# teoremma/pgen-rs

Hardware: AMD Instinct MI355X
Metric: genotypes decoded/sec (variants x samples / s) (higher is better)
Workload: dtype u8

## Files before the change

include/pgen_hip.h:

```cpp
#ifndef PGEN_HIP_H
#define PGEN_HIP_H

#include <stddef.h>
#include <stdint.h>

#ifdef __cplusplus
extern "C" {
#endif

#define PGENHIP_ABI_VERSION 2u
#define PGENHIP_LAUNCHES_IN_FLIGHT 16u

typedef enum pgenhip_status {
    PGENHIP_OK = 0,
    PGENHIP_ERR_BAD_ARG = -1,
    PGENHIP_ERR_HIP = -2,
    PGENHIP_ERR_OOM = -3,
    PGENHIP_ERR_INDEX_RANGE = -4,
    PGENHIP_ERR_BAD_MAGIC = -5,
    PGENHIP_ERR_BAD_MODE = -6,
    PGENHIP_ERR_BAD_FLAGS = -7,
    PGENHIP_ERR_NO_DEVICE = -8,
    PGENHIP_ERR_TOO_LARGE = -9,
    PGENHIP_ERR_IO = -10,
// ... 59 lines not shown

int pgenhip_decode_emit_at(pgenhip_ctx *ctx, const void *d_base, const uint64_t *d_record_off, uint32_t n_variants,
                           void *d_out, uint64_t out_stride, uint32_t flags);

int pgenhip_emit_lines(pgenhip_ctx *ctx, const void *d_records, uint64_t record_stride,
                       const uint32_t *d_variant_idx, uint32_t n_variants,
                       const void *d_prefix_blob, const uint64_t *d_prefix_off,
                       const uint64_t *d_line_off, uint64_t max_prefix_bytes,
                       void *d_out, uint32_t flags);

#define PGENHIP_COUNT_AUTO 0u
#define PGENHIP_COUNT_WAVE_PER_ROW 1u
#define PGENHIP_COUNT_ROWS_PER_WAVE 2u
int pgenhip_genotype_counts(pgenhip_ctx *ctx, const void *d_records, uint64_t record_stride, const uint32_t *d_variant_idx,
                            uint32_t n_variants, uint32_t *d_counts, uint32_t flags);
int pgenhip_genotype_counts_at(pgenhip_ctx *ctx, const void *d_base, const uint64_t *d_record_off, uint32_t n_variants,
                               uint32_t *d_counts, uint32_t flags);

#define PGENHIP_SCOUNT_AUTO 0u
#define PGENHIP_SCOUNT_ROWS 2u
#define PGENHIP_SCOUNT_SHAPE_MASK 0xFu
#define PGENHIP_SCOUNT_ACCUMULATE 0x10u
int pgenhip_sample_counts(pgenhip_ctx *ctx, const void *d_records, uint64_t record_stride, const uint32_t *d_variant_idx,
                          uint32_t n_variants, uint32_t *d_counts, uint32_t flags);
int pgenhip_sample_counts_at(pgenhip_ctx *ctx, const void *d_base, const uint64_t *d_record_off, uint32_t n_variants,
                             uint32_t *d_counts, uint32_t flags);

#define PGENHIP_MATRIX_AUTO 0u
#define PGENHIP_MATRIX_GENERAL 1u
#define PGENHIP_MATRIX_STREAM 2u
#define PGENHIP_MATRIX_TILE 3u
#define PGENHIP_MATRIX_SHAPE_MASK 0xFu
#define PGENHIP_MATRIX_SAMPLE_MAJOR 0x10u
int pgenhip_decode_matrix(pgenhip_ctx *ctx, const void *d_records, uint64_t record_stride, const uint32_t *d_variant_idx,
                          uint32_t n_variants, void *d_out, uint64_t out_stride, uint32_t elem_bytes,
                          const void *code_values, uint32_t flags);
int pgenhip_decode_matrix_at(pgenhip_ctx *ctx, const void *d_base, const uint64_t *d_record_off, uint32_t n_variants,
                             void *d_out, uint64_t out_stride, uint32_t elem_bytes, const void *code_values, uint32_t flags);

typedef enum pgenhip_knob {
    PGENHIP_KNOB_WIDE_BLOCKS_PER_CU = 1,
    PGENHIP_KNOB_WIDE_RANGES = 2,
    PGENHIP_KNOB_FLAT_BLOCKS_PER_CU = 3,
    PGENHIP_KNOB_SCAN_BLOCKS_PER_CU = 4,
    PGENHIP_KNOB_PICK_BATCH_BYTES = 6,
    PGENHIP_KNOB_SCAN_XCD_MAP = 8,
    PGENHIP_KNOB_SCAN_TWO_PASS = 9,
    PGENHIP_KNOB_SCAN_CHUNK_ROWS = 10,
    PGENHIP_KNOB_ROWPICK_BLOCKS_PER_CU = 11,
    PGENHIP_KNOB_SCAN_ROWPICK = 12,
    PGENHIP_KNOB_ALIGN_STORES = 16,
    PGENHIP_KNOB_SCOUNT_SLICES = 17,
    PGENHIP_KNOB_MATRIX_BLOCKS = 18,
    PGENHIP_KNOB_RUNS_ROWS = 7
} pgenhip_knob;
int pgenhip_tune(pgenhip_ctx *ctx, uint32_t knob, int32_t value);

int pgenhip_wait(pgenhip_ctx *ctx);

int pgenhip_timer_start(pgenhip_ctx *ctx);
int pgenhip_timer_stop(pgenhip_ctx *ctx, float *elapsed_ms);
int pgenhip_timer_mark(pgenhip_ctx *ctx);
int pgenhip_timer_read(pgenhip_ctx *ctx, float *elapsed_ms);

int pgenhip_device_malloc(pgenhip_ctx *ctx, void **d_ptr, size_t bytes);
int pgenhip_device_free(pgenhip_ctx *ctx, void *d_ptr);
int pgenhip_host_malloc_pinned(pgenhip_ctx *ctx, void **h_ptr, size_t bytes);
int pgenhip_host_free_pinned(pgenhip_ctx *ctx, void *h_ptr);
int pgenhip_memcpy_h2d(pgenhip_ctx *ctx, void *d_dst, const void *h_src, size_t bytes);
int pgenhip_memcpy_d2h(pgenhip_ctx *ctx, void *h_dst, const void *d_src, size_t bytes);

#define PGENHIP_SYNTH_DIRTY_PAD 1u
#define PGENHIP_SYNTH_HWE 2u
int pgenhip_synth_records(pgenhip_ctx *ctx, void *d_dst, uint64_t record_stride,
                          uint64_t first_variant, uint32_t n_variants,
                          uint64_t seed, uint32_t flags);

#ifdef __cplusplus
}
#endif
#endif
```

pgen_rs_amd/_capi.py:

```python
from __future__ import annotations

import ctypes as C
from pathlib import Path

import torch

PKG_DIR = Path(__file__).resolve().parent
LIB_PATH = PKG_DIR / "libpgen_hip.so"

OK = 0
ERR_BAD_ARG = -1
ERR_HIP = -2
ERR_OOM = -3
ERR_INDEX_RANGE = -4
ERR_BAD_MAGIC = -5
ERR_BAD_MODE = -6
ERR_BAD_FLAGS = -7
ERR_NO_DEVICE = -8
ERR_TOO_LARGE = -9
ERR_IO = -10
ERR_BAD_INDEX = -11
ERR_COMPRESSED_RECORD = -12

KERNEL_AUTO = 0
KERNEL_ROWS = 1
KERNEL_FLAT = 2
KERNEL_SCAN = 3
KERNEL_WIDE = 4
KERNEL_PICK = 6
KERNEL_RUNS = 7
KERNEL_ROWPICK = 8
COUNT_AUTO = 0
COUNT_WAVE_PER_ROW = 1
COUNT_ROWS_PER_WAVE = 2

SCOUNT_AUTO = 0
SCOUNT_ROWS = 2
SCOUNT_SHAPE_MASK = 0xF
SCOUNT_ACCUMULATE = 0x10
MATRIX_AUTO = 0
MATRIX_GENERAL = 1
MATRIX_STREAM = 2
MATRIX_TILE = 3
MATRIX_SHAPE_MASK = 0xF
MATRIX_SAMPLE_MAJOR = 0x10
SYNTH_DIRTY_PAD = 1
SYNTH_HWE = 2
CREATE_KEEP_LIST = 1
LAUNCHES_IN_FLIGHT = 16

KNOB_WIDE_BLOCKS_PER_CU = 1
KNOB_WIDE_RANGES = 2
KNOB_FLAT_BLOCKS_PER_CU = 3
KNOB_SCAN_BLOCKS_PER_CU = 4
KNOB_PICK_BATCH_BYTES = 6
KNOB_RUNS_ROWS = 7
KNOB_SCAN_XCD_MAP = 8
KNOB_SCAN_TWO_PASS = 9
KNOB_SCAN_CHUNK_ROWS = 10
KNOB_ROWPICK_BLOCKS_PER_CU = 11
KNOB_SCAN_ROWPICK = 12
KNOB_ALIGN_STORES = 16
KNOB_SCOUNT_SLICES = 17
KNOB_MATRIX_BLOCKS = 18



class VwHeader(C.Structure):
    _fields_ = [("variant_count", C.c_uint32), ("sample_count", C.c_uint32), ("storage_mode", C.c_uint8),
                ("record_type_bits", C.c_uint8), ("record_length_bytes", C.c_uint8), ("allele_count_bytes", C.c_uint8),
                ("provisional_ref_storage", C.c_uint8), ("reserved", C.c_uint8 * 3), ("block_count", C.c_uint64),
                ("main_header_body_offset", C.c_uint64), ("variant_records_offset", C.c_uint64)]


u8p = C.POINTER(C.c_uint8)
u32p = C.POINTER(C.c_uint32)
u64p = C.POINTER(C.c_uint64)
ctx_p = C.c_void_p

PROTOTYPES = {
    "pgenhip_abi_version": (C.c_uint32, []),
    "pgenhip_strerror": (C.c_char_p, [C.c_int]),
    "pgenhip_last_error_detail": (C.c_char_p, []),
    "pgenhip_device_count": (C.c_int, [C.POINTER(C.c_int)]),
    "pgenhip_variant_record_size": (C.c_uint32, [C.c_uint32]),
    "pgenhip_parse_header": (C.c_int, [C.c_char_p, u32p, u32p]),
    "pgenhip_record_offset": (C.c_uint64, [C.c_uint64, C.c_uint32]),
    "pgenhip_shard_range": (C.c_int, [C.c_uint64, C.c_uint32, C.c_uint32, u64p, u64p]),
    "pgenhip_vw_parse_header": (C.c_int, [C.c_char_p, C.POINTER(VwHeader)]),
    "pgenhip_vw_walk_index": (C.c_int, [C.POINTER(VwHeader), C.c_void_p, C.c_uint64, C.c_void_p, C.c_void_p, C.c_void_p]),
    "pgenhip_vw_select_uncompressed": (C.c_int, [C.c_void_p, C.c_void_p, C.c_void_p, C.c_uint32, C.c_void_p, C.c_uint32, C.c_uint32, C.c_void_p]),
    "pgenhip_create": (C.c_int, [C.POINTER(ctx_p), C.c_int, C.c_uint32, C.c_void_p, C.c_uint32, C.c_uint32]),
    "pgenhip_destroy": (C.c_int, [ctx_p]),
    "pgenhip_set_stream": (C.c_int, [ctx_p, C.c_void_p]),
    "pgenhip_reset_stream": (C.c_int, [ctx_p]),
    "pgenhip_sample_count": (C.c_uint32, [ctx_p]),
    "pgenhip_kept_count": (C.c_uint32, [ctx_p]),
    "pgenhip_gt_row_bytes": (C.c_uint64, [ctx_p]),
    "pgenhip_decode_emit": (C.c_int, [ctx_p, C.c_void_p, C.c_uint64, C.c_void_p, C.c_uint32, C.c_void_p, C.c_uint64, C.c_uint32]),
    "pgenhip_decode_emit_at": (C.c_int, [ctx_p, C.c_void_p, C.c_void_p, C.c_uint32, C.c_void_p, C.c_uint64, C.c_uint32]),
    "pgenhip_emit_lines": (C.c_int, [ctx_p, C.c_void_p, C.c_uint64, C.c_void_p, C.c_uint32, C.c_void_p, C.c_void_p, C.c_void_p, C.c_uint64, C.c_void_p, C.c_uint32]),
    "pgenhip_genotype_counts": (C.c_int, [ctx_p, C.c_void_p, C.c_uint64, C.c_void_p, C.c_uint32, C.c_void_p, C.c_uint32]),
    "pgenhip_genotype_counts_at": (C.c_int, [ctx_p, C.c_void_p, C.c_void_p, C.c_uint32, C.c_void_p, C.c_uint32]),
    "pgenhip_sample_counts": (C.c_int, [ctx_p, C.c_void_p, C.c_uint64, C.c_void_p, C.c_uint32, C.c_void_p, C.c_uint32]),
    "pgenhip_sample_counts_at": (C.c_int, [ctx_p, C.c_void_p, C.c_void_p, C.c_uint32, C.c_void_p, C.c_uint32]),
    "pgenhip_decode_matrix": (C.c_int, [ctx_p, C.c_void_p, C.c_uint64, C.c_void_p, C.c_uint32, C.c_void_p, C.c_uint64, C.c_uint32, C.c_void_p, C.c_uint32]),
    "pgenhip_decode_matrix_at": (C.c_int, [ctx_p, C.c_void_p, C.c_void_p, C.c_uint32, C.c_void_p, C.c_uint64, C.c_uint32, C.c_void_p, C.c_uint32]),
    "pgenhip_tune": (C.c_int, [ctx_p, C.c_uint32, C.c_int32]),
    "pgenhip_wait": (C.c_int, [ctx_p]),
    "pgenhip_timer_start": (C.c_int, [ctx_p]),
    "pgenhip_timer_stop": (C.c_int, [ctx_p, C.POINTER(C.c_float)]),
    "pgenhip_timer_mark": (C.c_int, [ctx_p]),
    "pgenhip_timer_read": (C.c_int, [ctx_p, C.POINTER(C.c_float)]),
    "pgenhip_device_malloc": (C.c_int, [ctx_p, C.POINTER(C.c_void_p), C.c_size_t]),
    "pgenhip_device_free": (C.c_int, [ctx_p, C.c_void_p]),
    "pgenhip_host_malloc_pinned": (C.c_int, [ctx_p, C.POINTER(C.c_void_p), C.c_size_t]),
    "pgenhip_host_free_pinned": (C.c_int, [ctx_p, C.c_void_p]),
# ... 35 lines not shown
```

pgen_rs_amd/csrc/capi.hip:

```cpp
#include "../../include/pgen_hip.h"

#include <algorithm>
#include <hip/hip_runtime.h>

#include <new>
#include <string>
#include <vector>

#include "host_pure.h"
#include "kernels.h"

using namespace pgenhip;

struct pgenhip_ctx {
    int device = 0;
    int num_cus = 256;
    uint32_t sample_count = 0;
    uint32_t record_size = 0;
    uint32_t kept_count = 0;
    bool subset = false;
    bool identity = false;
    uint32_t *d_kept = nullptr;
    uint8_t *d_count_mask = nullptr;
    uint32_t *d_scount_rank = nullptr;
// ... 616 lines not shown
        if (code_values) {
            const uint8_t *p = static_cast<const uint8_t *>(code_values) + (size_t)c * elem_bytes;
            v = 0u;
            for (uint32_t b = 0; b < elem_bytes; b++) v |= (uint32_t)p[b] << (8u * b);
        }
        a.tab[c] = v;
    }
    if (shape == PGENHIP_MATRIX_TILE && !gt_matrix_tile_applicable(a))
        return fail(PGENHIP_ERR_BAD_ARG, "PGENHIP_MATRIX_TILE needs d_out and out_stride to be multiples of 16 bytes");
    const int blocks = ctx->tune.matrix_blocks;
    if (shape == PGENHIP_MATRIX_STREAM || (shape == PGENHIP_MATRIX_AUTO && gt_matrix_stream_applicable(a)))
        HIP_TRY(launch_gt_matrix_stream(a, blocks, ctx->num_cus, ctx->stream));
    else if (shape == PGENHIP_MATRIX_TILE || (shape == PGENHIP_MATRIX_AUTO && gt_matrix_tile_applicable(a)))
        HIP_TRY(launch_gt_matrix_tile(a, blocks, ctx->num_cus, ctx->stream));
    else
        HIP_TRY(launch_gt_matrix_general(a, blocks, ctx->num_cus, ctx->stream));
    return PGENHIP_OK;
}

int pgenhip_decode_matrix(pgenhip_ctx *ctx, const void *d_records, uint64_t record_stride, const uint32_t *d_variant_idx,
                          uint32_t n_variants, void *d_out, uint64_t out_stride, uint32_t elem_bytes,
                          const void *code_values, uint32_t flags)
{
    return decode_matrix_core(ctx, d_records, record_stride, d_variant_idx, nullptr, n_variants, d_out, out_stride, elem_bytes, code_values, flags);
}

int pgenhip_decode_matrix_at(pgenhip_ctx *ctx, const void *d_base, const uint64_t *d_record_off, uint32_t n_variants,
                             void *d_out, uint64_t out_stride, uint32_t elem_bytes, const void *code_values, uint32_t flags)
{
    if (const int rc = check_record_off(ctx, d_record_off, n_variants)) return rc;
    return decode_matrix_core(ctx, d_base, 0, nullptr, d_record_off, n_variants, d_out, out_stride, elem_bytes, code_values, flags);
}

int pgenhip_tune(pgenhip_ctx *ctx, uint32_t knob, int32_t value)
{
    if (!ctx) return fail(PGENHIP_ERR_BAD_ARG, "ctx is NULL");
    const Tuning d;
    Tuning &t = ctx->tune;
    switch (knob) {
        case PGENHIP_KNOB_WIDE_BLOCKS_PER_CU: t.wide_blocks_per_cu = value > 0 ? value : d.wide_blocks_per_cu; break;
        case PGENHIP_KNOB_WIDE_RANGES:
            if (value < 0 || value > (int32_t)kMaxQueueRanges || (value & (value - 1)) != 0) return fail(PGENHIP_ERR_BAD_ARG, "ranges must be a power of two up to 64");
            t.wide_ranges = value ? value : d.wide_ranges;
            break;
        case PGENHIP_KNOB_FLAT_BLOCKS_PER_CU: t.flat_blocks_per_cu = value > 0 ? value : d.flat_blocks_per_cu; break;
        case PGENHIP_KNOB_SCAN_BLOCKS_PER_CU: t.scan_blocks_per_cu = value > 0 ? value : d.scan_blocks_per_cu; break;
        case PGENHIP_KNOB_PICK_BATCH_BYTES: t.pick_batch_bytes = value > 0 ? value : d.pick_batch_bytes; break;
        case PGENHIP_KNOB_SCAN_XCD_MAP: t.scan_xcd_map = value < 0 ? 0 : 1; break;
        case PGENHIP_KNOB_SCAN_CHUNK_ROWS: t.scan_chunk_rows = value > 0 ? value : d.scan_chunk_rows; break;
        case PGENHIP_KNOB_SCAN_TWO_PASS: t.scan_two_pass = value < 0 ? 0 : 1; break;
        case PGENHIP_KNOB_ROWPICK_BLOCKS_PER_CU: t.rowpick_blocks_per_cu = value > 0 ? value : d.rowpick_blocks_per_cu; break;
        case PGENHIP_KNOB_SCAN_ROWPICK: t.scan_rowpick = value < 0 ? 0 : 1; break;
        case PGENHIP_KNOB_ALIGN_STORES: t.align_stores = value < 0 ? 0 : 1; break;
        case PGENHIP_KNOB_RUNS_ROWS: t.runs_rows = value > 0 ? value : d.runs_rows; break;
        case PGENHIP_KNOB_SCOUNT_SLICES: t.scount_slices = value > 0 ? value : d.scount_slices; break;
        case PGENHIP_KNOB_MATRIX_BLOCKS: t.matrix_blocks = value > 0 ? value : d.matrix_blocks; break;
        default: return fail(PGENHIP_ERR_BAD_ARG, "unknown knob");
    }
    return PGENHIP_OK;
}

int pgenhip_wait(pgenhip_ctx *ctx)
{
    int rc = bind(ctx);
    if (rc) return rc;
    HIP_TRY(hipStreamSynchronize(ctx->stream));
    return PGENHIP_OK;
}

int pgenhip_timer_start(pgenhip_ctx *ctx)
{
    int rc = bind(ctx);
    if (rc) return rc;
    HIP_TRY(hipEventRecord(ctx->ev_start, ctx->stream));
    return PGENHIP_OK;
}

int pgenhip_timer_stop(pgenhip_ctx *ctx, float *elapsed_ms)
{
    int rc = bind(ctx);
    if (rc) return rc;
    if (!elapsed_ms) return fail(PGENHIP_ERR_BAD_ARG, "elapsed_ms is NULL");
    HIP_TRY(hipEventRecord(ctx->ev_stop, ctx->stream));
    HIP_TRY(hipEventSynchronize(ctx->ev_stop));
    HIP_TRY(hipEventElapsedTime(elapsed_ms, ctx->ev_start, ctx->ev_stop));
    return PGENHIP_OK;
}

int pgenhip_timer_mark(pgenhip_ctx *ctx)
{
    int rc = bind(ctx);
    if (rc) return rc;
    HIP_TRY(hipEventRecord(ctx->ev_stop, ctx->stream));
    return PGENHIP_OK;
}

int pgenhip_timer_read(pgenhip_ctx *ctx, float *elapsed_ms)
{
    int rc = bind(ctx);
    if (rc) return rc;
    if (!elapsed_ms) return fail(PGENHIP_ERR_BAD_ARG, "elapsed_ms is NULL");
    HIP_TRY(hipEventElapsedTime(elapsed_ms, ctx->ev_start, ctx->ev_stop));
    return PGENHIP_OK;
}

int pgenhip_device_malloc(pgenhip_ctx *ctx, void **d_ptr, size_t bytes)
// ... 73 lines not shown
```

pgen_rs_amd/csrc/gt_wide.hip:

```cpp
#include <algorithm>

#include "gt_common.hip.h"
#include "kernels.h"

namespace pgenhip {

namespace {

constexpr uint32_t kSpanChunks = 1024;
constexpr uint32_t kSlabBytes = 1088;
constexpr uint32_t kSlabExtra = 16;
constexpr uint32_t kDescBytes = 64;

struct WideParams {
    uint64_t row_bytes;
    uint64_t total_bytes;
    uint64_t n_items;
    uint32_t spans_per_row;
    uint32_t head;
    uint32_t n_ranges;
    uint32_t run_rows;
    uint32_t run_rec;
    uint32_t magic;
    uint32_t pfx_shift;
};

typedef uint32_t v4u __attribute__((ext_vector_type(4)));

template <bool HAS_VIDX>
__device__ __forceinline__ const uint8_t *row_record(const EmitArgs &a, uint64_t r)
{
    return HAS_VIDX ? gathered_record(a, r) : a.records + r * a.record_stride;
}

template <bool NT>
__device__ __forceinline__ void store_chunk(uint8_t *dst, const u32x4 &v)
{
    v4u t = {v.x, v.y, v.z, v.w};
    if (NT)
        __builtin_nontemporal_store(t, reinterpret_cast<v4u *>(dst));
    else
        *reinterpret_cast<v4u *>(dst) = t;
}

struct Item {
    uint64_t g0;
    uint32_t cnt;
    uint32_t lead;
    int64_t c_first;
    const uint8_t *rec;
    const uint8_t *base;
    uint32_t n_load;
    int32_t delta;
    uint64_t row;
    bool row_tail;
};

template <bool HAS_VIDX, bool LINES = false>
__device__ __forceinline__ Item make_item_at(const EmitArgs &a, const WideParams &p, uint64_t j, uint32_t k, uint64_t lines_row_start = 0ull,
                                             const uint8_t *rec_known = nullptr)
{
    Item it;
    const uint64_t S = p.row_bytes;
    const uint64_t row_start = LINES ? lines_row_start : j * S;
    const uint64_t g_first = (LINES || j == 0) ? (row_start + p.head) >> 4 : (row_start + p.head + 15ull) >> 4;
    const uint64_t g_end = (row_start + S + p.head + 15ull) >> 4;
    const int32_t row_chunks = (int32_t)(uint32_t)(g_end - g_first);
    const int32_t base_rel = (int32_t)(k * kSpanChunks) - (int32_t)((uint32_t)g_first & 63u);
    const int32_t end_rel = min(row_chunks, base_rel + (int32_t)kSpanChunks);
    const int32_t g0_rel = max(base_rel, 0);
    const int32_t row_c_first = (int32_t)((uint32_t)g_first * 16u - p.head - (uint32_t)row_start);
    it.row = j;
    it.g0 = g_first + (uint64_t)(uint32_t)g0_rel;
    it.cnt = end_rel > g0_rel ? (uint32_t)(end_rel - g0_rel) : 0u;
    it.lead = (uint32_t)(g0_rel - base_rel);
    it.row_tail = it.cnt != 0u && end_rel == row_chunks;
    it.c_first = (int64_t)row_c_first + ((int64_t)g0_rel << 4);
// ... 280 lines not shown
        for (uint32_t rr = rr_lo + lane; rr < rr_hi; rr += 64u) {
            const uint32_t e = rr * S + S - 1u;
            const uint32_t i = (uint32_t)((int32_t)e - c_first) >> 4;
            const uint32_t nl = (uint32_t)((int32_t)e - c_first) & 15u;
            const uint32_t slot = i + it.lead - g * 256u;
            const v4u x = st[slot];
            const bool has_next = rr + 1u < nrows || has_next_run;
            u32x4 y = {0u, 0u, 0u, 0u};
            if (nl < 15u && has_next) y = gt_text16_from_window((uint32_t)slab[delta + (rr + 1u) * R] << 8, -(int64_t)nl - 1);
            const uint32_t xs[4] = {x.x, x.y, x.z, x.w};
            const uint32_t ys[4] = {y.x, y.y, y.z, y.w};
            uint32_t os[4];
#pragma unroll
            for (int m = 0; m < 4; m++) {
                const int32_t nb = (int32_t)nl - 4 * m;
                const uint32_t mask = nb >= 4 ? 0xFFFFFFFFu : (nb <= 0 ? 0u : ((1u << (8 * nb)) - 1u));
                uint32_t d = (xs[m] & mask) | (ys[m] & ~mask);
                if (nb >= 0 && nb < 4) d = (d & ~(0xFFu << (8 * nb))) | (0x0Au << (8 * nb));
                os[m] = d;
            }
            if (has_next || nl == 15u) {
                st[slot] = v4u{os[0], os[1], os[2], os[3]};
            } else {
                uint8_t *const dst = chunk0 + (it.g0 + i) * 16ull;
#pragma unroll
                for (int b = 0; b < 16; b++)
                    if ((uint32_t)b <= nl) dst[b] = (uint8_t)(os[b >> 2] >> (8 * (b & 3)));
            }
        }
        __builtin_amdgcn_fence(__ATOMIC_RELEASE, "wavefront");
        __builtin_amdgcn_wave_barrier();
        __builtin_amdgcn_fence(__ATOMIC_ACQUIRE, "wavefront");
#pragma unroll
        for (uint32_t s4 = 0; s4 < 4u; s4++) {
            const uint32_t u = g * 4u + s4;
            if (u * 64u >= end) break;
            const uint32_t i = u * 64u + lane - it.lead;
            const v4u v = st[s4 * 64u + lane];
            if (i < cnt_whole && !(c_first < 0 && i == 0u)) store_chunk<NT>(span_ptr + u * 1024u, u32x4{v.x, v.y, v.z, v.w});
        }
        __builtin_amdgcn_fence(__ATOMIC_RELEASE, "wavefront");
        __builtin_amdgcn_wave_barrier();
    }
    if (c_first < 0 && it.cnt != 0u && lane < 16u && (int32_t)lane + c_first >= 0) {
        const uint32_t ob = (uint32_t)((int32_t)lane + c_first);
        const uint32_t code = ((uint32_t)slab[delta + (ob >> 4)] >> (((ob >> 2) & 3u) * 2u)) & 3u;
        chunk0[it.g0 * 16ull + lane] = (uint8_t)gt_text_byte(code, ob & 3u);
    }
}

constexpr int kRingSlots = 3;

template <int NS, bool HAS_VIDX, bool NT, bool LINES = false, int BURST = 2, bool RUNS = false>
__global__ __launch_bounds__(64 * (NS + 1)) void gt_stream_dyn_kernel(EmitArgs a, WideParams p)
{
    constexpr int RS = RUNS ? 2 : kRingSlots;
    constexpr int DS = RS + 1;
    __shared__ __attribute__((aligned(16))) uint8_t slabs[NS][RS][kSlabBytes + kSlabExtra];
    __shared__ __attribute__((aligned(16))) uint8_t s_desc[NS][DS][kDescBytes];
    __shared__ __attribute__((aligned(16))) uint8_t s_stage[RUNS ? NS : 1][RUNS ? kStageBytes : 16u];
    __shared__ uint32_t s_full[NS][RS];
    __shared__ uint32_t s_done[NS][RS];
    const uint32_t lane = threadIdx.x & 63u;
    const uint32_t wave = __builtin_amdgcn_readfirstlane(threadIdx.x >> 6);
    if (threadIdx.x < NS * RS) {
        (&s_full[0][0])[threadIdx.x] = 0u;
        (&s_done[0][0])[threadIdx.x] = 0u;
    }
    __syncthreads();
    constexpr uint64_t kNoItem = ~0ull;

    if (wave == 0u) {
        const uint32_t nr = p.n_ranges;
        const uint64_t per_range = (p.n_items + (uint64_t)nr - 1ull) / (uint64_t)nr;
        uint32_t range = blockIdx.x & (nr - 1u);
        uint32_t drained = 0u;
        auto issue_claim = [&](uint32_t rng) -> uint64_t {
            uint64_t got = 0;
            if (lane == 0u) got = atomicAdd(reinterpret_cast<unsigned long long *>(a.work_counters + rng * 16u), (unsigned long long)NS);
            return got;
        };
        uint64_t pending = issue_claim(range);
        for (uint32_t step = 0;; step++) {
            uint64_t t0 = kNoItem;
            uint64_t got = sgpr64(pending);
            while (drained < nr) {
                const uint64_t lo = (uint64_t)range * per_range;
                const uint64_t hi = min(lo + per_range, p.n_items);
                if (lo + got < hi) {
                    t0 = lo + got;
                    break;
                }
                range = (range + 1u) & (nr - 1u);
                drained++;
                if (drained < nr) got = sgpr64(issue_claim(range));
            }
            const uint64_t t_end = t0 == kNoItem ? 0ull : min(t0 + NS, min(((uint64_t)range + 1ull) * per_range, p.n_items));
            const uint32_t slot = (uint32_t)(step % RS);
            v4u in0[NS];
            v4u ext = v4u{0u, 0u, 0u, 0u};
            const uint8_t *ext_addr = a.records;
            bool ext_on = false;
            uint32_t nb[NS];
            uint64_t j_it = 0ull;
            uint32_t k_it = 0u;
            if (!RUNS && t0 != kNoItem) {
                j_it = p.spans_per_row == 1u ? t0 : t0 / p.spans_per_row;
                k_it = p.spans_per_row == 1u ? 0u : (uint32_t)(t0 - j_it * p.spans_per_row);
            }
            const uint32_t n_here = t0 == kNoItem ? 0u : (uint32_t)(t_end - t0);
            const uint64_t j_step = j_it;
            uint32_t rs_lo = 0u, rs_hi = 0u;
            if (LINES && t0 != kNoItem) {
                const uint64_t jr = min(j_it + (uint64_t)lane, (uint64_t)a.n_variants);
                const uint64_t lo_v = a.line_off[jr];
                const uint64_t po_v = a.prefix_off[jr];
                const uint64_t po_next = __shfl_down((unsigned long long)po_v, 1, 64);
                const uint64_t rs = lo_v + (po_next - po_v);
                asm volatile("v_mov_b32 %0, %2\n\tv_mov_b32 %1, %3" : "=v"(rs_lo), "=v"(rs_hi) : "v"((uint32_t)rs), "v"((uint32_t)(rs >> 32)));
            }
            uint32_t go_lo = 0u, go_hi = 0u;
            if (HAS_VIDX && !RUNS && t0 != kNoItem) {
                const uint64_t jr = min(j_it + (uint64_t)lane, (uint64_t)a.n_variants - 1ull);
                const uint64_t off = gathered_offset(a, jr);
                asm volatile("v_mov_b32 %1, %3\n\tv_mov_b32 %0, %2" : "=v"(go_lo), "=v"(go_hi) : "v"((uint32_t)off), "v"((uint32_t)(off >> 32)));
            }
            auto gathered_at = [&](uint32_t r) -> const uint8_t * {
                const uint32_t hi = (uint32_t)__builtin_amdgcn_readlane((int)go_hi, (int)r);
                const uint32_t lo = (uint32_t)__builtin_amdgcn_readlane((int)go_lo, (int)r);
                return a.records + (((uint64_t)hi << 32) | (uint64_t)lo);
            };
#pragma unroll
            for (int w = 0; w < NS; w++) {
                nb[w] = 0u;
                in0[w] = v4u{0u, 0u, 0u, 0u};
                if ((uint32_t)w >= n_here) {
                    if (lane == 0u) desc_put_item(s_desc[w][step % DS], Item{}, t0 == kNoItem ? kNoItem - 1ull : kNoItem);
                } else {
                    uint64_t row_start = 0ull;
                    if (LINES) {
                        const uint32_t r = (uint32_t)(j_it - j_step);
                        const uint32_t hi = (uint32_t)__builtin_amdgcn_readlane((int)rs_hi, (int)r);
                        const uint32_t lo = (uint32_t)__builtin_amdgcn_readlane((int)rs_lo, (int)r);
                        row_start = ((uint64_t)hi << 32) | (uint64_t)lo;
                    }
                    const uint32_t r_it = (uint32_t)(j_it - j_step);
                    const uint8_t *const rec_next = HAS_VIDX ? gathered_at(r_it + 1u) : nullptr;
                    const Item it = RUNS ? make_run_item(a, p, t0 + (uint64_t)w)
                                         : make_item_at<HAS_VIDX, LINES>(a, p, j_it, k_it, row_start, HAS_VIDX ? gathered_at(r_it) : nullptr);
                    if (!RUNS && ++k_it == p.spans_per_row) {
                        k_it = 0u;
                        j_it++;
                    }
                    if (lane == 0u) desc_put_item(s_desc[w][step % DS], it, t0 + (uint64_t)w);
                    if (lane < it.n_load) in0[w] = *reinterpret_cast<const v4u *>(it.base + lane * 16u);
                    if ((lane >> 1) == (uint32_t)w) {
                        ext_addr = it.base + (64u + (lane & 1u)) * 16u;
                        ext_on = 64u + (lane & 1u) < it.n_load;
                    }
                    if (!LINES && !RUNS && it.row_tail && (uint32_t)it.row + 1u < a.n_variants && lane == 0u)
                        nb[w] = (uint32_t)(HAS_VIDX ? rec_next : row_record<HAS_VIDX>(a, it.row + 1ull))[0];
                }
            }
            if (ext_on) ext = *reinterpret_cast<const v4u *>(ext_addr);
            if (t0 != kNoItem) pending = issue_claim(range);
#pragma unroll
            for (int w = 0; w < NS; w++) {
                if (step >= (uint32_t)RS) {
                    const uint32_t want = step - (uint32_t)RS + 1u;
                    while (lds_flag_read(lds_offset(&s_done[w][slot])) != want) __builtin_amdgcn_s_sleep(1);
                }
                uint8_t *slab = slabs[w][slot];
                *reinterpret_cast<v4u *>(slab + lane * 16u) = in0[w];
                if ((lane >> 1) == (uint32_t)w) *reinterpret_cast<v4u *>(slab + (64u + (lane & 1u)) * 16u) = ext;
                if (lane == 0u) slab[kSlabBytes] = (uint8_t)nb[w];
                if (lane == 0u) lds_flag_write(lds_offset(&s_full[w][slot]), step + 1u);
            }
            if (t0 == kNoItem) break;
        }
        {
            unsigned long long *const exits = reinterpret_cast<unsigned long long *>(a.work_counters + kMaxQueueRanges * 16u);
            uint32_t last = 0u;
            if (lane == 0u) last = atomicAdd(exits, 1ull) == (unsigned long long)gridDim.x - 1ull ? 1u : 0u;
            if (__builtin_amdgcn_readfirstlane(last)) {
                if (lane < kMaxQueueRanges) atomicExch(reinterpret_cast<unsigned long long *>(a.work_counters + lane * 16u), 0ull);
                if (lane == 0u) atomicExch(exits, 0ull);
            }
        }
    } else {
        const uint32_t w = wave - 1u;
        if (LINES && p.pfx_shift != 0u) copy_prefix_rows(a, p.pfx_shift, (uint64_t)blockIdx.x * NS + w, (uint64_t)gridDim.x * NS, lane);
        for (uint32_t step = 0;; step++) {
            const uint32_t slot = step % RS;
            while (lds_flag_read(lds_offset(&s_full[w][slot])) != step + 1u) __builtin_amdgcn_s_sleep(1);
            const uint8_t *slab = slabs[w][slot];
            const uint8_t *desc = s_desc[w][step % DS];
            uint64_t t = *reinterpret_cast<const uint64_t *>(desc + 8u);
            t = sgpr64(t);
            if (t == kNoItem - 1ull) break;
            if (t != kNoItem) {
                const Item it = desc_get_item(desc);
                if (RUNS)
                    emit_run<NT>(a, p, it, slab, s_stage[RUNS ? w : 0u], lane);
                else
                    emit_item<HAS_VIDX, NT, true, LINES, BURST>(a, p, it, slab, lane);
            }
            if (lane == 0u) lds_flag_write(lds_offset(&s_done[w][slot]), step + 1u);
        }
    }
}


constexpr uint32_t kLrMaxRows = 30;
constexpr uint32_t kLrRecBytes = kSlabBytes;
constexpr uint32_t kLrPfxBytes = 768;
constexpr uint32_t kLrSlab = kLrRecBytes + kLrPfxBytes + 2u * 32u * 4u;

__device__ __forceinline__ uint32_t run_text_byte(const uint8_t *slab, uint32_t rec_off, uint32_t x)
{
    const uint32_t code = ((uint32_t)slab[rec_off + (x >> 4)] >> (((x >> 2) & 3u) * 2u)) & 3u;
    return gt_text_byte(code, x & 3u);
}

constexpr uint32_t kTabFront = 4, kTabBack = 12, kTabMaxSamples = 4096;
__device__ __forceinline__ uint32_t tab_code(const uint8_t *rec, const uint16_t *tab, int32_t rank)
{
    const uint32_t s = (uint32_t)tab[rank];
    return ((uint32_t)rec[s >> 2] >> ((s & 3u) * 2u)) & 3u;
}

__device__ __forceinline__ u32x4 tab_text16(const uint8_t *rec, const uint16_t *tab, int32_t x)
{
    const int32_t g = x >> 2;
    const uint32_t sh = (uint32_t)x & 3u;
    const uint32_t t0 = gt_text(tab_code(rec, tab, g)), t1 = gt_text(tab_code(rec, tab, g + 1)), t2 = gt_text(tab_code(rec, tab, g + 2));
    const uint32_t t3 = gt_text(tab_code(rec, tab, g + 3)), t4 = gt_text(tab_code(rec, tab, g + 4));
    return u32x4{funnel_bytes(t0, t1, sh), funnel_bytes(t1, t2, sh), funnel_bytes(t2, t3, sh), funnel_bytes(t3, t4, sh)};
}

template <bool PICK>
__device__ __forceinline__ void emit_lines_run(const EmitArgs &a, const WideParams &p, const Item &it, const uint8_t *slab, uint8_t *stage,
                                               uint32_t pdelta, uint32_t lane, const uint16_t *tab)
{
    const int32_t N4 = (int32_t)(4u * a.kept_count);
    const uint32_t R = a.record_size;
    const uint32_t delta = (uint32_t)it.delta;
    const uint8_t *const pfx = slab + kLrRecBytes + pdelta;
    const uint32_t *const lrel = reinterpret_cast<const uint32_t *>(slab + kLrRecBytes + kLrPfxBytes);
    const uint32_t *const prel = lrel + 32;
    const uint32_t nrows = (uint32_t)min((uint64_t)p.run_rows, (uint64_t)a.n_variants - it.row);
    const bool has_next = it.row + (uint64_t)nrows < (uint64_t)a.n_variants;
    const int32_t run_len = (int32_t)lrel[nrows];
    uint8_t *const chunk0 = a.out - p.head;
    const int32_t c_first = (int32_t)it.c_first;
    uint8_t *const span_ptr = chunk0 + (it.g0 - it.lead) * 16ull + lane * 16u;
    const uint32_t end = it.lead + it.cnt;
    auto adown = [&](int32_t x) { return x - ((x - c_first) & 15); };
    auto aup = [&](int32_t x) { return x + ((c_first - x) & 15); };
    const int32_t own_end = c_first + 16 * (int32_t)it.cnt;
    const bool ragged_head = c_first < 0;
// ... 243 lines not shown
                        const uint64_t l0 = (uint64_t)__shfl((unsigned long long)lo_v[w], 0, 64), p0 = (uint64_t)__shfl((unsigned long long)po_v[w], 0, 64);
                        uint32_t *offs = reinterpret_cast<uint32_t *>(slab + kLrRecBytes + kLrPfxBytes);
                        offs[lane] = (uint32_t)(lo_v[w] - l0);
                        offs[32u + lane] = (uint32_t)(po_v[w] - p0);
                    }
                }
                if (lane == 0u) lds_flag_write(lds_offset(&s_full[w][slot]), step + 1u);
            }
            if (t0 == kNoItem) break;
        }
        {
            unsigned long long *const exits = reinterpret_cast<unsigned long long *>(a.work_counters + kMaxQueueRanges * 16u);
            uint32_t last = 0u;
            if (lane == 0u) last = atomicAdd(exits, 1ull) == (unsigned long long)gridDim.x - 1ull ? 1u : 0u;
            if (__builtin_amdgcn_readfirstlane(last)) {
                if (lane < kMaxQueueRanges) atomicExch(reinterpret_cast<unsigned long long *>(a.work_counters + lane * 16u), 0ull);
                if (lane == 0u) atomicExch(exits, 0ull);
            }
        }
    } else {
        const uint32_t w = wave - 1u;
        for (uint32_t step = 0;; step++) {
            const uint32_t slot = step % RS;
            while (lds_flag_read(lds_offset(&s_full[w][slot])) != step + 1u) __builtin_amdgcn_s_sleep(1);
            const uint8_t *slab = slabs[w][slot];
            const uint8_t *desc = s_desc[w][step % DS];
            uint64_t t = *reinterpret_cast<const uint64_t *>(desc + 8u);
            t = sgpr64(t);
            if (t == kNoItem - 1ull) break;
            if (t != kNoItem) {
                const Item it = desc_get_item(desc);
                const uint32_t pdelta = sgpr32(*reinterpret_cast<const uint32_t *>(desc + 52));
                emit_lines_run<PICK>(a, p, it, slab, s_stage[w], pdelta, lane, s_tab + (PICK ? kTabFront : 0u));
            }
            if (lane == 0u) lds_flag_write(lds_offset(&s_done[w][slot]), step + 1u);
        }
    }
}

}

bool gt_wide_applicable(const EmitArgs &a)
{
    return a.kept_idx == nullptr && a.line_off == nullptr && a.sample_count >= 1024u &&
           (a.n_variants <= 1 || a.out_stride == 4ull * a.kept_count + 1ull);
}

bool gt_wide_lines_applicable(const EmitArgs &a)
{
    return a.kept_idx == nullptr && a.line_off != nullptr && a.prefix_off != nullptr && a.sample_count >= 1024u &&
           a.work_counters != nullptr;
}

hipError_t launch_gt_wide(const EmitArgs &a, const Tuning &t, int num_cus, hipStream_t stream)
{
    if (a.n_variants == 0) return hipSuccess;
    if (a.work_counters == nullptr) return hipErrorInvalidValue;
    WideParams p;
    p.row_bytes = 4ull * a.kept_count + 1ull;
    p.total_bytes = (uint64_t)a.n_variants * p.row_bytes;
    p.head = (uint32_t)(((uint64_t)(uintptr_t)a.out) & 127ull);
    p.run_rows = 0u;
    p.run_rec = 0u;
    p.magic = 0u;
    p.pfx_shift = 0u;
    const uint64_t max_row_chunks = (p.row_bytes + 15ull) / 16ull + 1ull + 63ull;
    p.spans_per_row = (uint32_t)((max_row_chunks + kSpanChunks - 1ull) / kSpanChunks);
    p.n_items = (uint64_t)a.n_variants * p.spans_per_row;

    const uint64_t need = (p.n_items + 6ull) / 7ull;
    void (*dk)(EmitArgs, WideParams);
    if (a.line_off)
        dk = gathered(a) ? gt_stream_dyn_kernel<7, true, true, true> : gt_stream_dyn_kernel<7, false, true, true>;
    else
        dk = gathered(a) ? gt_stream_dyn_kernel<7, true, true> : gt_stream_dyn_kernel<7, false, true>;
    int per_cu = 0;
    if (hipOccupancyMaxActiveBlocksPerMultiprocessor(&per_cu, dk, 512, 0) != hipSuccess || per_cu < 1) per_cu = 2;
    if ((uint64_t)a.n_variants * p.row_bytes <= 1000000000ull && per_cu > 2) per_cu = 2;
    if (t.wide_blocks_per_cu > 0) per_cu = t.wide_blocks_per_cu;
    const uint64_t cap = (uint64_t)num_cus * (uint64_t)per_cu;
    const uint32_t g = (uint32_t)(need < cap ? need : cap);
    p.n_ranges = t.wide_ranges > 0 ? (uint32_t)t.wide_ranges : (p.spans_per_row > 1u && need >= 64ull * g ? 8u : 2u);
    p.pfx_shift = prefix_copy_shift(a);
    hipLaunchKernelGGL(dk, dim3(g), dim3(512), 0, stream, a, p);
    return hipGetLastError();
}

static uint32_t run_rows_for(const EmitArgs &a)
{
    if (a.record_size == 0u) return 0u;
    const uint32_t S = 4u * a.kept_count + 1u;
    const uint32_t by_load = 1040u / a.record_size;
    const uint32_t by_span = 15328u / S;
    return by_load < by_span ? by_load : by_span;
}

bool gt_runs_applicable(const EmitArgs &a)
{
    return a.kept_idx == nullptr && a.line_off == nullptr && !gathered(a) && a.sample_count >= 8u &&
           (a.n_variants <= 1 || (a.out_stride == 4ull * a.kept_count + 1ull && a.record_stride == a.record_size)) &&
           a.work_counters != nullptr && run_rows_for(a) >= 1u;
}

bool gt_runs_preferred(const EmitArgs &a) { return gt_runs_applicable(a) && run_rows_for(a) >= 2u; }

hipError_t launch_gt_runs(const EmitArgs &a, const Tuning &t, int num_cus, hipStream_t stream)
{
    if (a.n_variants == 0) return hipSuccess;
    if (!gt_runs_applicable(a)) return hipErrorInvalidValue;
    WideParams p;
    p.row_bytes = 4ull * a.kept_count + 1ull;
    p.total_bytes = (uint64_t)a.n_variants * p.row_bytes;
    p.head = (uint32_t)(((uint64_t)(uintptr_t)a.out) & 127ull);
    p.n_ranges = t.wide_ranges > 0 ? (uint32_t)t.wide_ranges : 2u;
    p.spans_per_row = 1u;
    p.run_rows = t.runs_rows > 0 && (uint32_t)t.runs_rows < run_rows_for(a) ? (uint32_t)t.runs_rows : run_rows_for(a);
    p.run_rec = a.record_size;
    p.magic = (uint32_t)(0x100000000ull / p.row_bytes) + 1u;
    p.pfx_shift = 0u;
    p.n_items = ((uint64_t)a.n_variants + p.run_rows - 1ull) / p.run_rows;
    const uint64_t need = (p.n_items + 6ull) / 7ull;
    void (*dk)(EmitArgs, WideParams) = gt_stream_dyn_kernel<7, false, true, false, 2, true>;
    int per_cu = 2;
    if (t.wide_blocks_per_cu > 0) per_cu = t.wide_blocks_per_cu;
    const uint64_t cap = (uint64_t)num_cus * (uint64_t)per_cu;
    hipLaunchKernelGGL(dk, dim3((uint32_t)(need < cap ? need : cap)), dim3(512), 0, stream, a, p);
    return hipGetLastError();
}

static uint32_t lineruns_rows_for(const EmitArgs &a)
{
    if (a.record_size == 0u || a.max_line_bytes == 0ull || a.max_line_bytes > 15328ull) return 0u;
    const uint32_t row_text = 4u * a.kept_count + 1u;
    const uint32_t max_prefix = (uint32_t)a.max_line_bytes - row_text;
    uint32_t b = 1040u / a.record_size;
    if (a.kept_idx && b) b--;
    b = std::min<uint32_t>(b, 15328u / (uint32_t)a.max_line_bytes);
    b = std::min<uint32_t>(b, kLrMaxRows);
    if (max_prefix) b = std::min<uint32_t>(b, (kLrPfxBytes - 16u) / max_prefix - (((kLrPfxBytes - 16u) / max_prefix) ? 1u : 0u));
    return b;
}

uint32_t gt_lineruns_rows(const EmitArgs &a) { return lineruns_rows_for(a); }

bool gt_lineruns_applicable(const EmitArgs &a)
{
    const bool samples_ok = a.kept_idx == nullptr ? a.sample_count >= 8u : (a.sample_count <= kTabMaxSamples && a.kept_count >= 8u);
    return samples_ok && a.line_off != nullptr && a.prefix_off != nullptr && !gathered(a) &&
           (a.n_variants <= 1 || a.record_stride == a.record_size) && a.work_counters != nullptr && lineruns_rows_for(a) >= 2u;
}

hipError_t launch_gt_lineruns(const EmitArgs &a, const Tuning &t, int num_cus, hipStream_t stream)
{
    if (a.n_variants == 0) return hipSuccess;
    if (!gt_lineruns_applicable(a)) return hipErrorInvalidValue;
    WideParams p;
    p.row_bytes = 4ull * a.kept_count + 1ull;
    p.total_bytes = 0ull;
    p.head = (uint32_t)(((uint64_t)(uintptr_t)a.out) & 127ull);
    p.n_ranges = t.wide_ranges > 0 ? (uint32_t)t.wide_ranges : 2u;
    p.spans_per_row = 1u;
    const uint32_t b_max = lineruns_rows_for(a);
    p.run_rows = t.runs_rows > 0 && (uint32_t)t.runs_rows < b_max ? (uint32_t)t.runs_rows : b_max;
    p.run_rec = a.record_size;
    p.magic = 0u;
    p.pfx_shift = 0u;
    p.n_items = ((uint64_t)a.n_variants + p.run_rows - 1ull) / p.run_rows;
    constexpr int kStorers = 3;
    const uint64_t need = (p.n_items + (uint64_t)kStorers - 1ull) / (uint64_t)kStorers;
    void (*dk)(EmitArgs, WideParams) = a.kept_idx ? gt_lineruns_kernel<kStorers, true> : gt_lineruns_kernel<kStorers, false>;
    constexpr int threads = 64 * (kStorers + 1);
    int per_cu = 0;
    if (hipOccupancyMaxActiveBlocksPerMultiprocessor(&per_cu, dk, threads, 0) != hipSuccess || per_cu < 1) per_cu = 1;
    if (t.wide_blocks_per_cu > 0) per_cu = t.wide_blocks_per_cu;
    const uint64_t cap = (uint64_t)num_cus * (uint64_t)per_cu;
    hipLaunchKernelGGL(dk, dim3((uint32_t)(need < cap ? need : cap)), dim3(threads), 0, stream, a, p);
    return hipGetLastError();
}

}
```

pgen_rs_amd/csrc/kernels.h:

```cpp
#pragma once
#include <hip/hip_runtime.h>
#include <stdint.h>

namespace pgenhip {

struct RowSource {
    const uint8_t *records;
    uint64_t record_stride;
    const uint32_t *variant_idx;
    const uint64_t *record_off;
    uint32_t n_variants;
    uint32_t sample_count;
    uint32_t record_size;
};

struct EmitArgs : RowSource {
    const uint32_t *kept_idx;
    uint32_t kept_count;
    uint8_t *out;
    uint64_t out_stride;
    const uint8_t *prefix_blob;
    const uint64_t *prefix_off;
    const uint64_t *line_off;
    uint64_t max_line_bytes;
    uint64_t *work_counters;
};

constexpr uint32_t kMaxQueueRanges = 64;

struct Tuning {
    int wide_blocks_per_cu = 0;
    int wide_ranges = 0;
    int flat_blocks_per_cu = 64;
    int scan_blocks_per_cu = 0;
    int pick_batch_bytes = 32768;
    int scan_xcd_map = 1;
    int scan_chunk_rows = 0;
    int scan_two_pass = 1;
    int rowpick_blocks_per_cu = 0;
    int scan_rowpick = 1;
    int align_stores = 1;
    int runs_rows = 0;
    int scount_slices = 0;
    int matrix_blocks = 0;
};

__host__ __device__ inline bool gathered(const RowSource &a) { return a.variant_idx != nullptr || a.record_off != nullptr; }

hipError_t launch_gt_rows(const EmitArgs &a, int num_cus, hipStream_t stream);

bool gt_flat_applicable(const EmitArgs &a);
hipError_t launch_gt_flat(const EmitArgs &a, const Tuning &t, int num_cus, hipStream_t stream);

bool gt_wide_applicable(const EmitArgs &a);
bool gt_wide_lines_applicable(const EmitArgs &a);
hipError_t launch_gt_wide(const EmitArgs &a, const Tuning &t, int num_cus, hipStream_t stream);
bool gt_runs_applicable(const EmitArgs &a);
bool gt_runs_preferred(const EmitArgs &a);
hipError_t launch_gt_runs(const EmitArgs &a, const Tuning &t, int num_cus, hipStream_t stream);
bool gt_lineruns_applicable(const EmitArgs &a);
uint32_t gt_lineruns_rows(const EmitArgs &a);
hipError_t launch_gt_lineruns(const EmitArgs &a, const Tuning &t, int num_cus, hipStream_t stream);

constexpr uint32_t kScanSegmentSamples = 16384u;
struct ScanArgs {
    const uint32_t *seg_rank;
    uint32_t max_seg_count;
    uint32_t align_stores;
};
constexpr uint32_t kCompactMaxSegCodes = 4096u;
hipError_t launch_gt_scan(const EmitArgs &a, const ScanArgs &sc, const Tuning &t, int num_cus, hipStream_t stream, bool compact = false);

constexpr uint32_t kRowPickMaxKept = 16384u;
bool gt_rowpick_applicable(const EmitArgs &a, int num_cus);
uint32_t gt_rowpick_resident_waves(const EmitArgs &a, const Tuning &t, int num_cus, bool compact);
hipError_t launch_gt_rowpick(const EmitArgs &a, const ScanArgs &sc, const Tuning &t, int num_cus, hipStream_t stream, bool compact = false);

bool gt_pick_applicable(const EmitArgs &a);
hipError_t launch_gt_pick(const EmitArgs &a, const Tuning &t, int num_cus, hipStream_t stream);

struct CountArgs : RowSource {
    uint32_t kept_count;
    const uint8_t *kept_mask;
    uint32_t *counts;
};
inline size_t gt_count_mask_bytes(uint32_t record_size) { return 16u * ((size_t)(record_size + 30u) / 16u + 2u); }
uint32_t gt_count_lanes_per_row(uint32_t record_size);
hipError_t launch_gt_count(const CountArgs &a, bool wave_per_row, int num_cus, hipStream_t stream);

struct ScountArgs : RowSource {
    const uint8_t *kept_mask;
    const uint32_t *kept_rank;
    uint32_t *counts;
};
// ... 26 lines not shown
```

Baseline: 1482 billion.

## Add static first claims and guided claim sizes to wide stream work queue

Changes the wide streaming kernel's dynamic scheduler so each block's first batch is assigned statically, without an atomic. Claim sizes can now shrink near the end of a range (guided scheduling) to balance the tail across blocks. Claimed items are rotated across storer waves via an index encoded in the LDS full-flag, so partial claims spread across waves. It adds per-claim arithmetic, an SGPR limit attribute and a new tuning knob, with default mode 1 enabling static-first claims, plus guided claims in the runs path.

```diff
diff --git a/include/pgen_hip.h b/include/pgen_hip.h
--- a/include/pgen_hip.h
+++ b/include/pgen_hip.h
@@ -135,6 +135,7 @@
     PGENHIP_KNOB_ALIGN_STORES = 16,
     PGENHIP_KNOB_SCOUNT_SLICES = 17,
     PGENHIP_KNOB_MATRIX_BLOCKS = 18,
+    PGENHIP_KNOB_WIDE_CLAIMS = 19,
     PGENHIP_KNOB_RUNS_ROWS = 7
 } pgenhip_knob;
 int pgenhip_tune(pgenhip_ctx *ctx, uint32_t knob, int32_t value);
diff --git a/pgen_rs_amd/_capi.py b/pgen_rs_amd/_capi.py
--- a/pgen_rs_amd/_capi.py
+++ b/pgen_rs_amd/_capi.py
@@ -63,6 +63,7 @@
 KNOB_ALIGN_STORES = 16
 KNOB_SCOUNT_SLICES = 17
 KNOB_MATRIX_BLOCKS = 18
+KNOB_WIDE_CLAIMS = 19
 
 
 
diff --git a/pgen_rs_amd/csrc/capi.hip b/pgen_rs_amd/csrc/capi.hip
--- a/pgen_rs_amd/csrc/capi.hip
+++ b/pgen_rs_amd/csrc/capi.hip
@@ -692,6 +692,10 @@
         case PGENHIP_KNOB_ROWPICK_BLOCKS_PER_CU: t.rowpick_blocks_per_cu = value > 0 ? value : d.rowpick_blocks_per_cu; break;
         case PGENHIP_KNOB_SCAN_ROWPICK: t.scan_rowpick = value < 0 ? 0 : 1; break;
         case PGENHIP_KNOB_ALIGN_STORES: t.align_stores = value < 0 ? 0 : 1; break;
+        case PGENHIP_KNOB_WIDE_CLAIMS:
+            if (value > 4) return fail(PGENHIP_ERR_BAD_ARG, "wide_claims: 1 .. 4 or -1");
+            t.wide_claims = value < 0 ? 0 : (value ? value : d.wide_claims);
+            break;
         case PGENHIP_KNOB_RUNS_ROWS: t.runs_rows = value > 0 ? value : d.runs_rows; break;
         case PGENHIP_KNOB_SCOUNT_SLICES: t.scount_slices = value > 0 ? value : d.scount_slices; break;
         case PGENHIP_KNOB_MATRIX_BLOCKS: t.matrix_blocks = value > 0 ? value : d.matrix_blocks; break;
diff --git a/pgen_rs_amd/csrc/gt_wide.hip b/pgen_rs_amd/csrc/gt_wide.hip
--- a/pgen_rs_amd/csrc/gt_wide.hip
+++ b/pgen_rs_amd/csrc/gt_wide.hip
@@ -23,6 +23,8 @@
     uint32_t run_rec;
     uint32_t magic;
     uint32_t pfx_shift;
+    uint32_t static_first;
+    uint32_t guided_claims;
 };
 
 typedef uint32_t v4u __attribute__((ext_vector_type(4)));
@@ -409,7 +411,7 @@
 constexpr int kRingSlots = 3;
 
 template <int NS, bool HAS_VIDX, bool NT, bool LINES = false, int BURST = 2, bool RUNS = false>
-__global__ __launch_bounds__(64 * (NS + 1)) void gt_stream_dyn_kernel(EmitArgs a, WideParams p)
+__global__ __launch_bounds__(64 * (NS + 1)) __attribute__((amdgpu_num_sgpr(102))) void gt_stream_dyn_kernel(EmitArgs a, WideParams p)
 {
     constexpr int RS = RUNS ? 2 : kRingSlots;
     constexpr int DS = RS + 1;
@@ -429,30 +431,69 @@
 
     if (wave == 0u) {
         const uint32_t nr = p.n_ranges;
-        const uint64_t per_range = (p.n_items + (uint64_t)nr - 1ull) / (uint64_t)nr;
         uint32_t range = blockIdx.x & (nr - 1u);
         uint32_t drained = 0u;
-        auto issue_claim = [&](uint32_t rng) -> uint64_t {
+        auto range_geom = [&](uint32_t q, uint64_t &base, uint64_t &avail, uint32_t &nblk) -> uint64_t {
+            const uint32_t nr_log2 = (uint32_t)__builtin_ctz(nr);
+            const uint64_t per_range = (p.n_items + (uint64_t)nr - 1ull) >> nr_log2;
+            const uint64_t lo = (uint64_t)q * per_range;
+            const uint64_t hi = min(lo + per_range, p.n_items);
+            const uint64_t len = hi > lo ? hi - lo : 0ull;
+            nblk = (gridDim.x + nr - 1u - q) >> nr_log2;
+            const uint64_t pre = p.static_first ? min((uint64_t)nblk * (uint64_t)NS, len) : 0ull;
+            base = lo + pre;
+            avail = len - pre;
+            return pre;
+        };
+        auto claim_size_for = [&](uint64_t rem, uint32_t nblk) -> uint32_t {
+            if (p.guided_claims == 0u) return (uint32_t)NS;
+            const uint32_t d = 2u * max(nblk, 1u);
+            if (rem > (uint64_t)d * (uint64_t)(NS - 1)) return (uint32_t)NS;
+            return max(((uint32_t)rem + d - 1u) / d, p.guided_claims);
+        };
+        auto issue_claim = [&](uint32_t rng, uint32_t size) -> uint64_t {
             uint64_t got = 0;
-            if (lane == 0u) got = atomicAdd(reinterpret_cast<unsigned long long *>(a.work_counters + rng * 16u), (unsigned long long)NS);
+            if (lane == 0u) got = atomicAdd(reinterpret_cast<unsigned long long *>(a.work_counters + rng * 16u), (unsigned long long)size);
             return got;
         };
-        uint64_t pending = issue_claim(range);
+        uint32_t claim_size = (uint32_t)NS;
+        uint64_t pending;
+        {
+            uint64_t base, avail;
+            uint32_t nblk;
+            const uint64_t pre = range_geom(range, base, avail, nblk);
+            const uint64_t s_first = (uint64_t)(blockIdx.x >> (uint32_t)__builtin_ctz(nr)) * (uint64_t)NS;
+            if (s_first < pre) {
+                pending = s_first - pre;
+            } else {
+                claim_size = claim_size_for(avail, nblk);
+                pending = issue_claim(range, claim_size);
+            }
+        }
+        uint32_t rot = 0u;
         for (uint32_t step = 0;; step++) {
             uint64_t t0 = kNoItem;
-            uint64_t got = sgpr64(pending);
+            uint64_t t_end = 0ull;
+            int64_t got = (int64_t)sgpr64(pending);
             while (drained < nr) {
-                const uint64_t lo = (uint64_t)range * per_range;
-                const uint64_t hi = min(lo + per_range, p.n_items);
-                if (lo + got < hi) {
-                    t0 = lo + got;
+                uint64_t base, avail;
+                uint32_t nblk;
+                range_geom(range, base, avail, nblk);
+                if (got < (int64_t)avail) {
+                    t0 = base + (uint64_t)got;
+                    t_end = min(t0 + (uint64_t)claim_size, base + avail);
+                    const int64_t used = (int64_t)(t_end - base);
+                    claim_size = claim_size_for(used > 0 ? avail - (uint64_t)used : avail, nblk);
                     break;
                 }
                 range = (range + 1u) & (nr - 1u);
                 drained++;
-                if (drained < nr) got = sgpr64(issue_claim(range));
-            }
-            const uint64_t t_end = t0 == kNoItem ? 0ull : min(t0 + NS, min(((uint64_t)range + 1ull) * per_range, p.n_items));
+                if (drained < nr) {
+                    range_geom(range, base, avail, nblk);
+                    claim_size = claim_size_for(avail, nblk);
+                    got = (int64_t)sgpr64(issue_claim(range, claim_size));
+                }
+            }
             const uint32_t slot = (uint32_t)(step % RS);
             v4u in0[NS];
             v4u ext = v4u{0u, 0u, 0u, 0u};
@@ -520,9 +561,10 @@
                 }
             }
             if (ext_on) ext = *reinterpret_cast<const v4u *>(ext_addr);
-            if (t0 != kNoItem) pending = issue_claim(range);
+            if (t0 != kNoItem) pending = issue_claim(range, claim_size);
 #pragma unroll
             for (int w = 0; w < NS; w++) {
+                const uint32_t sw = (uint32_t)w + rot >= (uint32_t)NS ? (uint32_t)w + rot - (uint32_t)NS : (uint32_t)w + rot;
                 if (step >= (uint32_t)RS) {
                     const uint32_t want = step - (uint32_t)RS + 1u;
                     while (lds_flag_read(lds_offset(&s_done[w][slot])) != want) __builtin_amdgcn_s_sleep(1);
@@ -531,9 +573,10 @@
                 *reinterpret_cast<v4u *>(slab + lane * 16u) = in0[w];
                 if ((lane >> 1) == (uint32_t)w) *reinterpret_cast<v4u *>(slab + (64u + (lane & 1u)) * 16u) = ext;
                 if (lane == 0u) slab[kSlabBytes] = (uint8_t)nb[w];
-                if (lane == 0u) lds_flag_write(lds_offset(&s_full[w][slot]), step + 1u);
+                if (lane == 0u) lds_flag_write(lds_offset(&s_full[0][slot]) + sw * (uint32_t)(RS * sizeof(uint32_t)), ((step + 1u) << 3) | (uint32_t)w);
             }
             if (t0 == kNoItem) break;
+            if (p.guided_claims) rot = (rot + n_here) % (uint32_t)NS;
         }
         {
             unsigned long long *const exits = reinterpret_cast<unsigned long long *>(a.work_counters + kMaxQueueRanges * 16u);
@@ -549,9 +592,11 @@
         if (LINES && p.pfx_shift != 0u) copy_prefix_rows(a, p.pfx_shift, (uint64_t)blockIdx.x * NS + w, (uint64_t)gridDim.x * NS, lane);
         for (uint32_t step = 0;; step++) {
             const uint32_t slot = step % RS;
-            while (lds_flag_read(lds_offset(&s_full[w][slot])) != step + 1u) __builtin_amdgcn_s_sleep(1);
-            const uint8_t *slab = slabs[w][slot];
-            const uint8_t *desc = s_desc[w][step % DS];
+            uint32_t full;
+            while (((full = lds_flag_read(lds_offset(&s_full[w][slot]))) >> 3) != step + 1u) __builtin_amdgcn_s_sleep(1);
+            const uint32_t wi = sgpr32(full) & 7u;
+            const uint8_t *slab = slabs[wi][slot];
+            const uint8_t *desc = s_desc[wi][step % DS];
             uint64_t t = *reinterpret_cast<const uint64_t *>(desc + 8u);
             t = sgpr64(t);
             if (t == kNoItem - 1ull) break;
@@ -562,7 +607,7 @@
                 else
                     emit_item<HAS_VIDX, NT, true, LINES, BURST>(a, p, it, slab, lane);
             }
-            if (lane == 0u) lds_flag_write(lds_offset(&s_done[w][slot]), step + 1u);
+            if (lane == 0u) lds_flag_write(lds_offset(&s_done[wi][slot]), step + 1u);
         }
     }
 }
@@ -912,6 +957,14 @@
            a.work_counters != nullptr;
 }
 
+static void set_claims(WideParams &p, const Tuning &t, bool runs)
+{
+    const int mode = t.wide_claims;
+    p.static_first = (mode == 1 || mode == 2 || mode == 4) ? 1u : 0u;
+    const bool guided = mode == 3 || mode == 4 || (mode == 1 && runs);
+    p.guided_claims = guided ? (runs ? 2u : 3u) : 0u;
+}
+
 hipError_t launch_gt_wide(const EmitArgs &a, const Tuning &t, int num_cus, hipStream_t stream)
 {
     if (a.n_variants == 0) return hipSuccess;
@@ -942,6 +995,7 @@
     const uint32_t g = (uint32_t)(need < cap ? need : cap);
     p.n_ranges = t.wide_ranges > 0 ? (uint32_t)t.wide_ranges : (p.spans_per_row > 1u && need >= 64ull * g ? 8u : 2u);
     p.pfx_shift = prefix_copy_shift(a);
+    set_claims(p, t, false);
     hipLaunchKernelGGL(dk, dim3(g), dim3(512), 0, stream, a, p);
     return hipGetLastError();
 }
@@ -984,6 +1038,7 @@
     int per_cu = 2;
     if (t.wide_blocks_per_cu > 0) per_cu = t.wide_blocks_per_cu;
     const uint64_t cap = (uint64_t)num_cus * (uint64_t)per_cu;
+    set_claims(p, t, true);
     hipLaunchKernelGGL(dk, dim3((uint32_t)(need < cap ? need : cap)), dim3(512), 0, stream, a, p);
     return hipGetLastError();
 }
@@ -1025,6 +1080,8 @@
     p.run_rec = a.record_size;
     p.magic = 0u;
     p.pfx_shift = 0u;
+    p.static_first = 0u;
+    p.guided_claims = 0u;
     p.n_items = ((uint64_t)a.n_variants + p.run_rows - 1ull) / p.run_rows;
     constexpr int kStorers = 3;
     const uint64_t need = (p.n_items + (uint64_t)kStorers - 1ull) / (uint64_t)kStorers;
diff --git a/pgen_rs_amd/csrc/kernels.h b/pgen_rs_amd/csrc/kernels.h
--- a/pgen_rs_amd/csrc/kernels.h
+++ b/pgen_rs_amd/csrc/kernels.h
@@ -40,6 +40,7 @@
     int rowpick_blocks_per_cu = 0;
     int scan_rowpick = 1;
     int align_stores = 1;
+    int wide_claims = 1;
     int runs_rows = 0;
     int scount_slices = 0;
     int matrix_blocks = 0;
```

Result: no change. 1480 billion (-0.2%).
